# gmarcais/Jellyfish

Measured on AMD Instinct MI355X. Metric: k-mers/sec at k=21 canonical, 150 bp synthetic reads, bit-exact counts, higher is better.
Workload: dtype u64

## Files before the change

### jellyfish_amd/csrc/kernels_tile.hip.hpp

```cpp
#pragma once
#include "kernels_part.hip.hpp"

namespace jfgpu {

__device__ __attribute__((noinline)) void ovf_add_call(uint64_t* ovf_key, uint64_t* ovf_cnt, uint64_t ovf_mask, uint64_t* counters,
                                                       uint64_t slot, uint64_t units) {
  DevTable V; V.ovf_key = ovf_key; V.ovf_cnt = ovf_cnt; V.ovf_mask = ovf_mask; V.counters = counters;
  ovf_add(V, slot, units);
}

#ifndef JFGPU_T_BLOCK
#define JFGPU_T_BLOCK 512
#endif
constexpr int kTileBlock = JFGPU_T_BLOCK;
constexpr uint32_t kQueueLook = 2;
#ifndef JFGPU_T_QUEUE
#define JFGPU_T_QUEUE 6144
#endif
constexpr uint32_t kTileQueueBytes = JFGPU_T_QUEUE;

inline size_t tile_rank_lds(size_t slot_bytes, uint32_t tile_bits, int tpb) {
  const size_t nslots = (size_t)tpb << tile_bits;
  return nslots * slot_bytes + (nslots >> kBucketBits) * 2 + 16 + kTileQueueBytes;
}

template <typename ITEM, bool RETURNING, typename SLOT, int TPB, int BLOCK = kTileBlock, bool HEAVY = false, bool SAMPLE = false>
__global__ __launch_bounds__(BLOCK, (BLOCK >= 512 ? 2 * BLOCK / 256 : 4)) void tile_rank_insert_kernel(DevTable T, SegList S, uint64_t tile0, uint32_t n_tiles) {
  constexpr int NP = ((sizeof(ITEM) == 8 || (BLOCK < 512 && TPB == 1)) ? 4608 : 9216) / BLOCK;
  constexpr uint32_t kVec = 16 / sizeof(SLOT);
  constexpr uint32_t kB = 1u << kBucketBits;
  constexpr uint32_t kBV = kB / kVec;
  constexpr uint32_t kSlotBits = 8 * sizeof(SLOT);
  JF_DYN_LDS(s_raw);
  const TableGeom& g = T.g;
  constexpr uint32_t tsz = 1u << kMaxTileBits, nslots = TPB * tsz, nbkt = nslots >> kBucketBits, tmask = tsz - 1;
  constexpr uint32_t NBK = nbkt / BLOCK;
  SLOT* const s_tile = reinterpret_cast<SLOT*>(s_raw);
  uint32_t* const s_cnt = reinterpret_cast<uint32_t*>(s_raw + (size_t)nslots * sizeof(SLOT));
  uint32_t* const s_qn = s_cnt + (nbkt >> 1);
  constexpr uint32_t qcap = kTileQueueBytes / sizeof(ITEM) / (BLOCK / 64);
  static_assert(qcap >= 64, "phase C stages one held-back item per lane through the queue");
  ITEM* const s_q = reinterpret_cast<ITEM*>(s_qn + 4) + (threadIdx.x >> 6) * qcap;
  SLOT* const gslots = reinterpret_cast<SLOT*>(T.slots);
  const SLOT lmask = (SLOT)g.low_mask, inc = (SLOT)g.inc, occ = (SLOT)g.occ_bit;
  const uint32_t cshift = g.tag_bits + 1, idshift = kSlotBits - cshift;
  const uint32_t lane = threadIdx.x & 63;
  const unsigned long long below = lane ? (~0ull >> (64 - lane)) : 0ull;
  const ITEM hole = (ITEM)~(ITEM)0;

  auto unit_dirty = [&](uint32_t t) -> uint32_t {
    if(TPB == 2) return *reinterpret_cast<const uint16_t*>(T.dirty + tile0 + 2 * (uint64_t)t);
    return T.dirty[tile0 + t];
  };
  auto zero_counters = [&]() {
    for(uint32_t i = threadIdx.x; i < (nbkt >> 1); i += BLOCK) s_cnt[i] = 0;
  };
  auto zero_tile = [&]() {
    for(uint32_t i = threadIdx.x * kVec; i < nslots; i += BLOCK * kVec) *reinterpret_cast<uint4*>(s_tile + i) = make_uint4(0, 0, 0, 0);
  };
  auto load_tile = [&](const SLOT* gt, uint32_t d) {
    for(uint32_t b = threadIdx.x; b < nbkt; b += BLOCK) {
      const bool ld = (d >> (8 * ((b << kBucketBits) >> kMaxTileBits))) & 0xFFu;
      uint32_t c = 0;
#pragma unroll
      for(uint32_t q = 0; q < kBV; ++q) {
        uint4 v = make_uint4(0, 0, 0, 0);
        if(ld) v = *reinterpret_cast<const uint4*>(gt + ((size_t)b << kBucketBits) + q * kVec);
        *reinterpret_cast<uint4*>(s_tile + ((size_t)b << kBucketBits) + q * kVec) = v;
        if(sizeof(SLOT) == 4) c += (v.x != 0) + (v.y != 0) + (v.z != 0) + (v.w != 0);
        else c += ((v.x | v.y) != 0) + ((v.z | v.w) != 0);
      }
      reinterpret_cast<uint16_t*>(s_cnt)[b] = (uint16_t)c;
    }
  };
  auto home_of = [&](ITEM x) -> uint32_t {
    if constexpr(sizeof(ITEM) == 4) return ((uint32_t)x >> g.rem_bits) & (nslots - 1);
    else return (uint32_t)((uint64_t)x >> g.rem_bits) & (nslots - 1);
  };
  auto load_bucket = [&](uint32_t bs, SLOT (&w)[kB]) {
#pragma unroll
    for(uint32_t q = 0; q < kBV; ++q) {
      const uint4 v = *reinterpret_cast<const uint4*>(s_tile + bs + q * kVec);
      if constexpr(sizeof(SLOT) == 4) { w[4 * q] = (SLOT)v.x; w[4 * q + 1] = (SLOT)v.y; w[4 * q + 2] = (SLOT)v.z; w[4 * q + 3] = (SLOT)v.w; }
      else { w[2 * q] = (SLOT)(((uint64_t)v.y << 32) | v.x); w[2 * q + 1] = (SLOT)(((uint64_t)v.w << 32) | v.z); }
    }
  };
  auto store_bucket = [&](uint32_t bs, const SLOT (&w)[kB]) {
#pragma unroll
    for(uint32_t q = 0; q < kBV; ++q) {
      uint4 v;
      if constexpr(sizeof(SLOT) == 4) v = make_uint4((uint32_t)w[4 * q], (uint32_t)w[4 * q + 1], (uint32_t)w[4 * q + 2], (uint32_t)w[4 * q + 3]);
      else v = make_uint4((uint32_t)w[2 * q], (uint32_t)((uint64_t)w[2 * q] >> 32), (uint32_t)w[2 * q + 1], (uint32_t)((uint64_t)w[2 * q + 1] >> 32));
      *reinterpret_cast<uint4*>(s_tile + bs + q * kVec) = v;
    }
  };
  auto has_dups = [&](const SLOT (&w)[kB]) -> bool {
    SLOT sh[kB];
#pragma unroll
    for(uint32_t i = 0; i < kB; ++i) sh[i] = w[i] << idshift;
    bool d = false;
#pragma unroll
    for(uint32_t j = 1; j < kB; ++j) {
      bool e = false;
#pragma unroll
      for(uint32_t i = 0; i < j; ++i) e = e | (sh[i] == sh[j]);
      d = d | (e & (w[j] != 0));
    }
    return d;
  };
  auto merge_bucket = [&](SLOT (&w)[kB], uint64_t bucket_slot0) {
    const SLOT cmask = (SLOT)g.cnt_max;
    SLOT carry[kB];
#pragma unroll
    for(uint32_t i = 0; i < kB; ++i) carry[i] = 0;
#pragma unroll
    for(uint32_t j = 1; j < kB; ++j)
#pragma unroll
      for(uint32_t i = 0; i < j; ++i) {
        const bool same = (w[j] != 0) & (w[i] != 0) & (((w[i] ^ w[j]) & lmask) == 0);
        const SLOT sum = (SLOT)(w[i] >> cshift) + (same ? (SLOT)(w[j] >> cshift) : (SLOT)0);
        w[i] = (w[i] & lmask) | (SLOT)((sum & cmask) << cshift);
        carry[i] += (SLOT)(sum >> g.cnt_bits);
        w[j] = same ? (SLOT)0 : w[j];
      }
    SLOT o[kB], oc[kB];
#pragma unroll
    for(uint32_t i = 0; i < kB; ++i) { o[i] = 0; oc[i] = 0; }
    uint32_t n = 0;
#pragma unroll
    for(uint32_t j = 0; j < kB; ++j) {
      const bool ne = w[j] != 0;
#pragma unroll
      for(uint32_t d = 0; d <= j; ++d) { const bool here = ne & (n == d); o[d] = here ? w[j] : o[d]; oc[d] = here ? carry[j] : oc[d]; }
      n += ne ? 1u : 0u;
    }
    SLOT any = 0;
#pragma unroll
    for(uint32_t q = 0; q < kB; ++q) { w[q] = o[q]; any |= oc[q]; }
    if(RETURNING && any != 0) {
#pragma unroll
      for(uint32_t q = 0; q < kB; ++q) if(oc[q]) ovf_add_call(T.ovf_key, T.ovf_cnt, T.ovf_mask, T.counters, bucket_slot0 + q, (uint64_t)oc[q]);
    }
  };
  auto merge_tile = [&](uint64_t unit_slot0) {
    constexpr uint32_t MB0 = (TPB == 2 && sizeof(ITEM) + sizeof(SLOT) == 8 && NBK >= 4) ? 4 : (NBK >= 2 ? 2 : 1);
    constexpr uint32_t Rmax = nbkt / (BLOCK / 64);
    static_assert(Rmax >= 128, "the merge list must fit the bucket counters");
    constexpr uint32_t R = Rmax >= 512 ? 512 : Rmax >= 256 ? 256 : 128;
    constexpr uint32_t MBr = R >= 512 ? 4 : R >= 256 ? 2 : 1;
    constexpr uint32_t MBw = 16 / kB >= 1 ? 16 / kB : 1;
    constexpr uint32_t MB = MB0 < MBr ? (MB0 < MBw ? MB0 : MBw) : (MBr < MBw ? MBr : MBw);
    static_assert((BLOCK / 64) * R * 2 <= nbkt * 2, "the merge list must fit the bucket counters");
    uint16_t* const lst = reinterpret_cast<uint16_t*>(s_cnt) + (threadIdx.x >> 6) * R;
    uint32_t head = 0, cnt = 0;
#pragma unroll 1
    for(uint32_t k0 = 0; k0 < NBK; k0 += MB) {
      SLOT wb[MB][kB];
#pragma unroll
      for(uint32_t k = 0; k < MB; ++k) load_bucket((threadIdx.x + (k0 + k) * BLOCK) << kBucketBits, wb[k]);
#pragma unroll
      for(uint32_t k = 0; k < MB; ++k) {
        const bool dup = has_dups(wb[k]);
        const unsigned long long m = __ballot(dup);
        if(dup) lst[(head + cnt + (uint32_t)__popcll(m & below)) & (R - 1)] = (uint16_t)(threadIdx.x + (k0 + k) * BLOCK);
        cnt += (uint32_t)__popcll(m);
      }
      const bool last = k0 + MB >= NBK;
      while(cnt >= 64 || (last && cnt)) {
        const uint32_t n = cnt < 64 ? cnt : 64;
        (void)__ballot(true);
        if(lane < n) {
          const uint32_t b = lst[(head + lane) & (R - 1)];
          SLOT w[kB];
          load_bucket(b << kBucketBits, w);
          merge_bucket(w, unit_slot0 + ((uint64_t)b << kBucketBits));
          store_bucket(b << kBucketBits, w);
        }
        head += n; cnt -= n;
      }
    }
  };
  auto store_tile = [&](SLOT* gt, uint32_t t) {
#pragma unroll
    for(uint32_t k = 0; k < NBK; ++k) {
      const uint32_t b = threadIdx.x + k * BLOCK;
#pragma unroll
      for(uint32_t q = 0; q < kBV; ++q) {
        const uint4 v = *reinterpret_cast<const uint4*>(s_tile + ((size_t)b << kBucketBits) + q * kVec);
        *reinterpret_cast<uint4*>(gt + ((size_t)b << kBucketBits) + q * kVec) = v;
        *reinterpret_cast<uint4*>(s_tile + ((size_t)b << kBucketBits) + q * kVec) = make_uint4(0, 0, 0, 0);
      }
    }
    zero_counters();
    if(threadIdx.x == 0) {
      if(TPB == 2) *reinterpret_cast<uint16_t*>(T.dirty + tile0 + 2 * (uint64_t)t) = 0x0101;
      else T.dirty[tile0 + t] = 1;
    }
  };
  auto slow_insert = [&](ITEM x, uint64_t unit_slot0) {
    constexpr uint32_t LK = kQueueLook;
    const SLOT low = occ | (SLOT)((uint64_t)x & (g.occ_bit - 1)), neww = inc | low;
    const uint32_t h = home_of(x), hbase = h & ~tmask, hb = h & tmask & ~(kB - 1u);
    const uint32_t max_steps = (T.max_probe >> kBucketBits) + 1;
    for(uint32_t step = 0; step < max_steps; ) {
      SLOT w[LK][kB];
#pragma unroll
      for(uint32_t k = 0; k < LK; ++k) load_bucket(hbase + ((hb + ((step + k) << kBucketBits)) & tmask), w[k]);
      uint32_t hitm = 0, empm = 0;
#pragma unroll
      for(uint32_t k = 0; k < LK; ++k)
#pragma unroll
        for(uint32_t i = 0; i < kB; ++i) {
          hitm |= (uint32_t)((w[k][i] & lmask) == low) << (kB * k + i);
          empm |= (uint32_t)(w[k][i] == 0) << (kB * k + i);
        }
      for(uint32_t cand = hitm | empm; cand; cand &= cand - 1) {
        const uint32_t j = (uint32_t)__ffs((int)cand) - 1u;
        if(step + (j >> kBucketBits) >= max_steps) { step = max_steps; break; }
        const uint32_t at = hbase + ((hb + (step << kBucketBits) + j) & tmask);
        bool add = (hitm >> j) & 1;
        if(!add) {
          const SLOT was = atomicCAS(&s_tile[at], (SLOT)0, neww);
          if(was == 0) return;
          add = (was & lmask) == low;
        }
        if(add) {
          if(RETURNING) {
            const SLOT prev = atomicAdd(&s_tile[at], inc);
            if(((uint64_t)prev >> cshift) + 1 > g.cnt_max) ovf_add_call(T.ovf_key, T.ovf_cnt, T.ovf_mask, T.counters, unit_slot0 + at, 1);
          } else atomicAdd(&s_tile[at], inc);
          return;
        }
      }
      step += LK;
    }
    atomicAdd((unsigned long long*)&T.counters[CTR_FULL], 1ull);
  };

  [[maybe_unused]] PhaseClk pc;
  auto rank_request = [&](const ITEM (&it)[NP], uint32_t vm, uint32_t (&old)[NP]) {
#pragma unroll
    for(int r = 0; r < NP; ++r)
      if((vm >> r) & 1) { const uint32_t b = home_of(it[r]) >> kBucketBits; old[r] = atomicAdd(&s_cnt[b >> 1], 1u << ((b & 1) * 16)); }
  };
  [[maybe_unused]] uint32_t smp_items = 0, smp_queued = 0;
  auto place_round = [&](ITEM (&it)[NP], uint32_t vm, const uint32_t (&old)[NP], uint64_t unit_slot0, const ITEM* again, auto&& after_a) {
    uint32_t qn = 0, pend = 0;
    [[maybe_unused]] uint32_t ovm = 0;
#pragma unroll
    for(int r = 0; r < NP; ++r) JF_OPAQUE(it[r]);
#pragma unroll
    for(int r = 0; r < NP; ++r) {
      bool ov = false;
      if((vm >> r) & 1) {
        const uint32_t b = home_of(it[r]) >> kBucketBits;
        const uint32_t rank = (old[r] >> ((b & 1) * 16)) & 0xFFFFu;
        if(rank < kB) s_tile[(b << kBucketBits) + rank] = inc | occ | (SLOT)((uint64_t)it[r] & (g.occ_bit - 1));
        else ov = true;
      }
      if constexpr(HEAVY) { if(ov) ovm |= 1u << r; }
      else {
        const unsigned long long m = __ballot(ov);
        if(ov) {
          const uint32_t at = qn + (uint32_t)__popcll(m & below);
          if(at < qcap) s_q[at] = it[r]; else pend |= 1u << r;
        }
        qn += (uint32_t)__popcll(m);
      }
    }
    if constexpr(SAMPLE) { smp_items += (uint32_t)__popc(vm); smp_queued += qn; }
    if constexpr(!HEAVY) after_a();
    lds_barrier();
    JF_PHASE(pc, 2);
    merge_tile(unit_slot0);
    lds_barrier();
    JF_PHASE(pc, 6);
    uint32_t nq = qn < qcap ? qn : qcap;
    if constexpr(HEAVY) {
      uint32_t q2 = 0, carry = 0;
      constexpr int CB = kB == 4 ? 6 : 3;
#pragma unroll
      for(int r0 = 0; r0 < NP; r0 += CB) {
        SLOT wb[CB][kB];
#pragma unroll
        for(int k = 0; k < CB; ++k)
          if(r0 + k < NP && ((ovm >> (r0 + k)) & 1)) load_bucket(home_of(it[r0 + k < NP ? r0 + k : 0]) & ~(kB - 1u), wb[k]);
#pragma unroll
        for(int k = 0; k < CB; ++k) {
          if(r0 + k >= NP) continue;
          const int r = r0 + k;
          bool miss = false;
          if((ovm >> r) & 1) {
            const ITEM x = it[r];
            const SLOT low = occ | (SLOT)((uint64_t)x & (g.occ_bit - 1));
            const uint32_t bs = home_of(x) & ~(kB - 1u);
            int hit = -1;
#pragma unroll
            for(int i = (int)kB - 1; i >= 0; --i) if((wb[k][i] & lmask) == low) hit = i;
            if(hit >= 0) {
              if(RETURNING) {
                const SLOT prev = atomicAdd(&s_tile[bs + hit], inc);
                if(((uint64_t)prev >> cshift) + 1 > g.cnt_max) carry |= 1u << r;
              } else atomicAdd(&s_tile[bs + hit], inc);
            } else miss = true;
          }
          const unsigned long long m2 = __ballot(miss);
          if(miss) {
            const uint32_t at = q2 + (uint32_t)__popcll(m2 & below);
            if(at < qcap) s_q[at] = it[r]; else pend |= 1u << r;
          }
          q2 += (uint32_t)__popcll(m2);
        }
      }
      (void)__ballot(true);
      after_a();
      while(carry) {
        const uint32_t r = (uint32_t)__ffs((int)carry) - 1u; carry &= carry - 1;
        const ITEM x = again[r * BLOCK + threadIdx.x];
        const SLOT low = occ | (SLOT)((uint64_t)x & (g.occ_bit - 1));
        const uint32_t bs = home_of(x) & ~(kB - 1u);
        SLOT w[kB];
        load_bucket(bs, w);
        uint32_t hit = 0;
#pragma unroll
        for(int i = (int)kB - 1; i >= 1; --i) if((w[i] & lmask) == low) hit = (uint32_t)i;
        if((w[0] & lmask) == low) hit = 0;
        ovf_add_call(T.ovf_key, T.ovf_cnt, T.ovf_mask, T.counters, unit_slot0 + bs + hit, 1);
      }
      nq = q2 < qcap ? q2 : qcap;
    }
    for(;;) {
      for(uint32_t i = lane; i < nq; i += 64) slow_insert(s_q[i], unit_slot0);
      const unsigned long long m = __ballot(pend != 0);
      if(!m) break;
      if(pend) {
        const uint32_t r = (uint32_t)__ffs((int)pend) - 1u;
        pend &= pend - 1;
        s_q[(uint32_t)__popcll(m & below)] = again[r * BLOCK + threadIdx.x];
      }
      nq = (uint32_t)__popcll(m);
      (void)__ballot(true);
    }
    JF_PHASE(pc, 5);
    lds_barrier();
    JF_PHASE(pc, 3);
  };
  zero_counters();
  zero_tile();
  lds_barrier();
  const uint64_t* off = S.off[0];
  const uint32_t sh = S.sh[0];
  const bool holes = sh != 0;
  const ITEM* src = reinterpret_cast<const ITEM*>(S.items[0]);
  const uint32_t G = gridDim.x;
  constexpr uint64_t kRound = (uint64_t)NP * BLOCK;
  uint32_t t = blockIdx.x;
  uint64_t a0 = 0, b0 = 0, a1 = 0, b1 = 0; uint32_t d0 = 0, d1 = 0;
  ITEM cur[NP];
  auto fetch = [&](uint64_t a, uint64_t b) {
    const ITEM* ub = src + a;
    const uint32_t n = (uint32_t)((b - a) < kRound ? (b - a) : kRound);
    if(b <= a) return;
    uint32_t tid = threadIdx.x;
    JF_OPAQUE(tid);
#pragma unroll
    for(int r = 0; r < NP; ++r) {
      const uint32_t i = (uint32_t)r * BLOCK + tid;
      cur[r] = ub[i < n ? i : n - 1];
    }
  };
  if(t < n_tiles) { a0 = off[(size_t)t << sh]; b0 = off[((size_t)t << sh) + 1]; d0 = unit_dirty(t); }
  if(t + G < n_tiles) { a1 = off[(size_t)(t + G) << sh]; b1 = off[((size_t)(t + G) << sh) + 1]; d1 = unit_dirty(t + G); }
  fetch(a0, b0);
  uint64_t c0 = a0;
  while(t < n_tiles) {
    if(b0 <= a0) {
      uint64_t a2 = 0, b2 = 0; uint32_t d2 = 0;
      if(t + 2 * G < n_tiles) { a2 = off[(size_t)(t + 2 * G) << sh]; b2 = off[((size_t)(t + 2 * G) << sh) + 1]; d2 = unit_dirty(t + 2 * G); }
      t += G; a0 = a1; b0 = b1; d0 = d1; a1 = a2; b1 = b2; d1 = d2; c0 = a0;
      fetch(a0, b0);
      continue;
    }
    const bool first = c0 == a0, last = c0 + kRound >= b0;
    const uint64_t unit_slot0 = (tile0 + (uint64_t)TPB * t) << kMaxTileBits;
    SLOT* gt = gslots + unit_slot0;
    JF_PHASE(pc, 0);
    const uint32_t n0 = (uint32_t)((b0 - c0) < kRound ? (b0 - c0) : kRound);
    uint32_t vm = 0, tid = threadIdx.x;
    JF_OPAQUE(tid);
#pragma unroll
    for(int r = 0; r < NP; ++r)
      if((uint32_t)r * BLOCK + tid < n0 && !(holes && cur[r] == hole)) vm |= 1u << r;
    const uint32_t d_eff = first ? d0 : (TPB == 2 ? 0x0101u : 1u);
    if(d_eff) { load_tile(gt, d_eff); lds_barrier(); }
    uint32_t old[NP];
    rank_request(cur, vm, old);
    JF_PHASE(pc, 1);
    uint64_t a2 = 0, b2 = 0; uint32_t d2 = 0;
    if(last && t + 2 * G < n_tiles) { a2 = off[(size_t)(t + 2 * G) << sh]; b2 = off[((size_t)(t + 2 * G) << sh) + 1]; d2 = unit_dirty(t + 2 * G); }
    place_round(cur, vm, old, unit_slot0, src + c0, [&] { if(last) fetch(a1, b1); else fetch(c0 + kRound, b0); });
    store_tile(gt, t);
    lds_barrier();
    JF_PHASE(pc, 4);
    if(last) { t += G; a0 = a1; b0 = b1; d0 = d1; a1 = a2; b1 = b2; d1 = d2; c0 = a0; }
    else c0 += kRound;
  }
  JF_PHASE_FLUSH(pc, 16);
  if constexpr(SAMPLE) {
    uint32_t w = smp_items;
    for(int o = 32; o > 0; o >>= 1) w += __shfl_down(w, o, 64);
    if(lane == 0) {
      atomicAdd((unsigned long long*)&T.counters[CTR_T_ITEMS], (unsigned long long)w);
      atomicAdd((unsigned long long*)&T.counters[CTR_T_QUEUED], (unsigned long long)smp_queued);
    }
  }
}

}
```

Baseline: 15.16 billion.

## Use buffer loads/stores with scalar offsets for tile and item transfers

Tile load/store and item fetch now go through AMDGPU buffer resource descriptors, with wave-uniform base addresses forced into scalar registers and per-row scalar offsets. This is meant to cut VGPR address arithmetic and 64-bit pointer math. Out-of-range item reads are clamped by the hardware bounds check instead of a per-element min. The per-round valid-item bitmask is replaced by a row count plus partial-row flag, which drops per-item comparisons but makes the validity test per row. There is a risk that out-of-bounds items now read as zero rather than the last item, which relies on the validity check to skip them.

```diff
diff --git a/jellyfish_amd/csrc/kernels_tile.hip.hpp b/jellyfish_amd/csrc/kernels_tile.hip.hpp
--- a/jellyfish_amd/csrc/kernels_tile.hip.hpp
+++ b/jellyfish_amd/csrc/kernels_tile.hip.hpp
@@ -8,6 +8,13 @@
   DevTable V; V.ovf_key = ovf_key; V.ovf_cnt = ovf_cnt; V.ovf_mask = ovf_mask; V.counters = counters;
   ovf_add(V, slot, units);
 }
+
+#if defined(JFGPU_EMU)
+__device__ __forceinline__ uint32_t uniform32(uint32_t x) { return x; }
+#else
+__device__ __forceinline__ uint32_t uniform32(uint32_t x) { x = (uint32_t)__builtin_amdgcn_readfirstlane((int)x); asm("" : "+s"(x)); return x; }
+#endif
+__device__ __forceinline__ uint64_t uniform64(uint64_t x) { return ((uint64_t)uniform32((uint32_t)(x >> 32)) << 32) | uniform32((uint32_t)x); }
 
 #ifndef JFGPU_T_BLOCK
 #define JFGPU_T_BLOCK 512
@@ -47,7 +54,26 @@
   const uint32_t lane = threadIdx.x & 63;
   const unsigned long long below = lane ? (~0ull >> (64 - lane)) : 0ull;
   const ITEM hole = (ITEM)~(ITEM)0;
-
+  constexpr uint32_t kRowBytes = BLOCK * kB * (uint32_t)sizeof(SLOT);
+  const uint32_t lane_off = threadIdx.x * (kB * (uint32_t)sizeof(SLOT));
+#if defined(JFGPU_EMU)
+  auto unit_ref = [&](const SLOT* gt) { return reinterpret_cast<unsigned char*>(const_cast<SLOT*>(gt)); };
+  auto unit_ld = [&](unsigned char* u, uint32_t voff, uint32_t soff) -> uint4 { return *reinterpret_cast<const uint4*>(u + voff + soff); };
+  auto unit_st = [&](unsigned char* u, uint32_t voff, uint32_t soff, uint4 v) { *reinterpret_cast<uint4*>(u + voff + soff) = v; };
+#else
+  typedef unsigned int u32x4 __attribute__((__vector_size__(16)));
+  auto unit_ref = [&](const SLOT* gt) {
+    return __builtin_amdgcn_make_buffer_rsrc(reinterpret_cast<void*>(uniform64((uint64_t)gt)), 0, (int)(nslots * sizeof(SLOT)), 0x00020000);
+  };
+  auto unit_ld = [&](__amdgpu_buffer_rsrc_t u, uint32_t voff, uint32_t soff) -> uint4 {
+    const u32x4 v = __builtin_amdgcn_raw_buffer_load_b128(u, (int)voff, (int)soff, 0);
+    return make_uint4(v[0], v[1], v[2], v[3]);
+  };
+  auto unit_st = [&](__amdgpu_buffer_rsrc_t u, uint32_t voff, uint32_t soff, uint4 v) {
+    const u32x4 w = {v.x, v.y, v.z, v.w};
+    __builtin_amdgcn_raw_buffer_store_b128(w, u, (int)voff, (int)soff, 0);
+  };
+#endif
   auto unit_dirty = [&](uint32_t t) -> uint32_t {
     if(TPB == 2) return *reinterpret_cast<const uint16_t*>(T.dirty + tile0 + 2 * (uint64_t)t);
     return T.dirty[tile0 + t];
@@ -59,14 +85,17 @@
     for(uint32_t i = threadIdx.x * kVec; i < nslots; i += BLOCK * kVec) *reinterpret_cast<uint4*>(s_tile + i) = make_uint4(0, 0, 0, 0);
   };
   auto load_tile = [&](const SLOT* gt, uint32_t d) {
-    for(uint32_t b = threadIdx.x; b < nbkt; b += BLOCK) {
+    const auto u = unit_ref(gt);
+#pragma unroll
+    for(uint32_t k = 0; k < NBK; ++k) {
+      const uint32_t b = threadIdx.x + k * BLOCK;
       const bool ld = (d >> (8 * ((b << kBucketBits) >> kMaxTileBits))) & 0xFFu;
       uint32_t c = 0;
 #pragma unroll
       for(uint32_t q = 0; q < kBV; ++q) {
         uint4 v = make_uint4(0, 0, 0, 0);
-        if(ld) v = *reinterpret_cast<const uint4*>(gt + ((size_t)b << kBucketBits) + q * kVec);
-        *reinterpret_cast<uint4*>(s_tile + ((size_t)b << kBucketBits) + q * kVec) = v;
+        if(ld) v = unit_ld(u, lane_off + q * 16u, k * kRowBytes);
+        *reinterpret_cast<uint4*>(s_raw + k * kRowBytes + lane_off + q * 16u) = v;
         if(sizeof(SLOT) == 4) c += (v.x != 0) + (v.y != 0) + (v.z != 0) + (v.w != 0);
         else c += ((v.x | v.y) != 0) + ((v.z | v.w) != 0);
       }
@@ -181,14 +210,15 @@
     }
   };
   auto store_tile = [&](SLOT* gt, uint32_t t) {
+    const auto u = unit_ref(gt);
 #pragma unroll
     for(uint32_t k = 0; k < NBK; ++k) {
-      const uint32_t b = threadIdx.x + k * BLOCK;
 #pragma unroll
       for(uint32_t q = 0; q < kBV; ++q) {
-        const uint4 v = *reinterpret_cast<const uint4*>(s_tile + ((size_t)b << kBucketBits) + q * kVec);
-        *reinterpret_cast<uint4*>(gt + ((size_t)b << kBucketBits) + q * kVec) = v;
-        *reinterpret_cast<uint4*>(s_tile + ((size_t)b << kBucketBits) + q * kVec) = make_uint4(0, 0, 0, 0);
+        uint4* const sp = reinterpret_cast<uint4*>(s_raw + k * kRowBytes + lane_off + q * 16u);
+        const uint4 v = *sp;
+        unit_st(u, lane_off + q * 16u, k * kRowBytes, v);
+        *sp = make_uint4(0, 0, 0, 0);
       }
     }
     zero_counters();
@@ -238,13 +268,18 @@
   };
 
   [[maybe_unused]] PhaseClk pc;
-  auto rank_request = [&](const ITEM (&it)[NP], uint32_t vm, uint32_t (&old)[NP]) {
+  struct Rows { uint32_t full; bool part, holes; };
+  auto is_item = [&](const Rows& v, ITEM x, int r) -> bool {
+    const bool row = (uint32_t)r < v.full ? true : ((uint32_t)r == v.full ? v.part : false);
+    return row & !(v.holes & (x == hole));
+  };
+  auto rank_request = [&](const ITEM (&it)[NP], const Rows& vm, uint32_t (&old)[NP]) {
 #pragma unroll
     for(int r = 0; r < NP; ++r)
-      if((vm >> r) & 1) { const uint32_t b = home_of(it[r]) >> kBucketBits; old[r] = atomicAdd(&s_cnt[b >> 1], 1u << ((b & 1) * 16)); }
+      if(is_item(vm, it[r], r)) { const uint32_t b = home_of(it[r]) >> kBucketBits; old[r] = atomicAdd(&s_cnt[b >> 1], 1u << ((b & 1) * 16)); }
   };
   [[maybe_unused]] uint32_t smp_items = 0, smp_queued = 0;
-  auto place_round = [&](ITEM (&it)[NP], uint32_t vm, const uint32_t (&old)[NP], uint64_t unit_slot0, const ITEM* again, auto&& after_a) {
+  auto place_round = [&](ITEM (&it)[NP], const Rows& vm, const uint32_t (&old)[NP], uint64_t unit_slot0, const ITEM* again, auto&& after_a) {
     uint32_t qn = 0, pend = 0;
     [[maybe_unused]] uint32_t ovm = 0;
 #pragma unroll
@@ -252,7 +287,9 @@
 #pragma unroll
     for(int r = 0; r < NP; ++r) {
       bool ov = false;
-      if((vm >> r) & 1) {
+      const bool valid = is_item(vm, it[r], r);
+      if constexpr(SAMPLE) smp_items += valid ? 1u : 0u;
+      if(valid) {
         const uint32_t b = home_of(it[r]) >> kBucketBits;
         const uint32_t rank = (old[r] >> ((b & 1) * 16)) & 0xFFFFu;
         if(rank < kB) s_tile[(b << kBucketBits) + rank] = inc | occ | (SLOT)((uint64_t)it[r] & (g.occ_bit - 1));
@@ -268,7 +305,7 @@
         qn += (uint32_t)__popcll(m);
       }
     }
-    if constexpr(SAMPLE) { smp_items += (uint32_t)__popc(vm); smp_queued += qn; }
+    if constexpr(SAMPLE) smp_queued += qn;
     if constexpr(!HEAVY) after_a();
     lds_barrier();
     JF_PHASE(pc, 2);
@@ -361,13 +398,31 @@
     const ITEM* ub = src + a;
     const uint32_t n = (uint32_t)((b - a) < kRound ? (b - a) : kRound);
     if(b <= a) return;
-    uint32_t tid = threadIdx.x;
-    JF_OPAQUE(tid);
+#if defined(JFGPU_EMU)
 #pragma unroll
     for(int r = 0; r < NP; ++r) {
-      const uint32_t i = (uint32_t)r * BLOCK + tid;
-      cur[r] = ub[i < n ? i : n - 1];
-    }
+      const uint32_t i = (uint32_t)r * BLOCK + threadIdx.x;
+      cur[r] = i < n ? ub[i] : (ITEM)0;
+    }
+#else
+    constexpr uint32_t kItemRow = BLOCK * (uint32_t)sizeof(ITEM);
+    constexpr int RG = kItemRow < 4096 ? (int)(4096 / kItemRow) : 1;
+    const uint32_t voff = threadIdx.x * (uint32_t)sizeof(ITEM);
+    const uint64_t ua = uniform64((uint64_t)ub);
+    const uint32_t have = uniform32(n) * (uint32_t)sizeof(ITEM);
+#pragma unroll
+    for(int r0 = 0; r0 < NP; r0 += RG) {
+      const int before = r0 * (int)kItemRow;
+      const int left = (int)have - before;
+      const auto rs = __builtin_amdgcn_make_buffer_rsrc(reinterpret_cast<void*>(ua + (uint32_t)before), 0, left > 0 ? left : 0, 0x00020000);
+#pragma unroll
+      for(int q = 0; q < RG; ++q) {
+        if(r0 + q >= NP) continue;
+        if constexpr(sizeof(ITEM) == 4) cur[r0 + q] = (ITEM)__builtin_amdgcn_raw_buffer_load_b32(rs, voff + (uint32_t)q * kItemRow, 0, 0);
+        else { const auto v = __builtin_amdgcn_raw_buffer_load_b64(rs, voff + (uint32_t)q * kItemRow, 0, 0); cur[r0 + q] = (ITEM)(((uint64_t)v[1] << 32) | v[0]); }
+      }
+    }
+#endif
   };
   if(t < n_tiles) { a0 = off[(size_t)t << sh]; b0 = off[((size_t)t << sh) + 1]; d0 = unit_dirty(t); }
   if(t + G < n_tiles) { a1 = off[(size_t)(t + G) << sh]; b1 = off[((size_t)(t + G) << sh) + 1]; d1 = unit_dirty(t + G); }
@@ -385,12 +440,8 @@
     const uint64_t unit_slot0 = (tile0 + (uint64_t)TPB * t) << kMaxTileBits;
     SLOT* gt = gslots + unit_slot0;
     JF_PHASE(pc, 0);
-    const uint32_t n0 = (uint32_t)((b0 - c0) < kRound ? (b0 - c0) : kRound);
-    uint32_t vm = 0, tid = threadIdx.x;
-    JF_OPAQUE(tid);
-#pragma unroll
-    for(int r = 0; r < NP; ++r)
-      if((uint32_t)r * BLOCK + tid < n0 && !(holes && cur[r] == hole)) vm |= 1u << r;
+    const uint32_t n0 = uniform32((uint32_t)((b0 - c0) < kRound ? (b0 - c0) : kRound));
+    const Rows vm = {n0 / BLOCK, threadIdx.x < n0 % BLOCK, holes};
     const uint32_t d_eff = first ? d0 : (TPB == 2 ? 0x0101u : 1u);
     if(d_eff) { load_tile(gt, d_eff); lds_barrier(); }
     uint32_t old[NP];
```

Result: no change. 15.18 billion (median of 3 runs) (+0.1%).
